# meilisearch/arroy

Measured on AMD Instinct MI355X. Metric: distances/sec, Q=1 batched 768-dim cosine scan (GB/s vs HBM roofline in `roofline`); tree-build seconds at 10M vectors in `build_10m`, higher is better.
Workload: dtype f32; 1 GPU; 1M x 768 cosine Q=1 scan (configs[1])

## Files before the change

### arroy_amd/csrc/api.hip

```cpp
#include <algorithm>
#include <atomic>
#include <chrono>
#include <cmath>
#include <condition_variable>
#include <functional>
#include <immintrin.h>
#include <new>
#include <thread>
#include <cctype>
#include <cstdio>
#include <mutex>
#include <vector>
#include <sched.h>
#include <sys/syscall.h>
#include <unistd.h>

#include "common.h"

namespace ah {

static thread_local std::string g_error;
static thread_local ah_error_detail g_detail = {AH_OK, 0, 0, 0};

static thread_local int g_guard_depth = 0;
// ... 1998 lines not shown
        std::lock_guard<std::mutex> lk(ds->mu);
        ah_rerank_stats &r = ds->rr_stats;
        r.calls += 1;
        r.queries += nq;
        r.candidates += total;
        r.seconds_wall += wall;
        r.seconds_prep += prep;
        r.seconds_ids += ids;
        r.seconds_enqueue += enqueue;
        r.seconds_sync_wait += wait;
        r.seconds_device_span += ms * 1e-3;
    }
};
#define AH_RR_SYNC(stream_)                       \
    do {                                          \
        probe.lap(&RerankProbe::enqueue);         \
        AH_HIP(hipStreamSynchronize(stream_));    \
        probe.lap(&RerankProbe::wait);            \
    } while (0)

static int rerank_batch_chunk(ah_dataset *ds, Context *ctx, const float *queries, size_t nq, const uint32_t *ids,
                              const uint64_t *offsets, size_t k, uint32_t *out_ids, float *out_distances,
                              uint32_t *out_counts) {
    const uint64_t base = offsets[0];
    const uint64_t total = offsets[nq] - base;
    RerankProbe probe(ds, ctx, nq, total);
    uint32_t max_n = 0, max_rounds = 0;
    std::vector<HostSeg> segs(nq);
    std::vector<HostTile> tiles;
    const uint32_t tc = batch_tile_candidates();
    for (size_t q = 0; q < nq; q++) {
        const uint64_t nq_items = offsets[q + 1] - offsets[q];
        AH_REQUIRE(nq_items < 0xFFFFFFFFull, AH_ERR_INVALID_ARGUMENT, "candidate list too long");
        segs[q] = HostSeg{offsets[q] - base, (uint32_t)nq_items, (uint32_t)std::min<uint64_t>(k, nq_items)};
        out_counts[q] = segs[q].k;
        max_n = std::max(max_n, segs[q].n);
        max_rounds = std::max(max_rounds, batch_rounds(segs[q].n, segs[q].k));
        for (uint32_t f = 0; f < segs[q].n; f += tc) tiles.push_back(HostTile{(uint32_t)q, f});
    }
    const size_t qstride = pad256(ds->row_bytes());
    const size_t kstride = batch_key_stride(std::max<uint32_t>(max_n, 1));
    const size_t inv_bytes = batch_invert_wanted(ds->view(), total) ? batch_invert_counter_bytes(ds->n, total) : 0;
    bool screened = tun(TUN_RERANK_SCREEN) != 0 && (ds->metric == AH_COSINE || ds->metric == AH_DOT_PRODUCT) && ds->dims >= 32 &&
                    inv_bytes == 0 && k <= 256 && total >= 8 * k * nq && !tiles.empty();
    if (screened) screened = ensure_screen(ds, ctx->stream, false);
    const bool screened8 = screened && tun(TUN_RERANK_SCREEN8) != 0 && !ds->rerank8_off.load(std::memory_order_relaxed) &&
                           ensure_screen8_search(ds, ctx->stream);
    const size_t screen_bytes = (screened ? pad256(nq * (size_t)ds->hpitch * 2) + pad256(nq * 16) + pad256(total * 4) : 0) +
                                (screened8 ? pad256(nq * (size_t)ds->pitch8 * 2) + pad256(nq * 16) + pad256(total * 4) : 0);
    const size_t dev_bytes = pad256(nq * (size_t)ds->dims * 4) + nq * qstride + pad256(nq * 8) + pad256(nq * sizeof(HostSeg)) +
                             pad256(tiles.size() * sizeof(HostTile)) + pad256(total * 4) * 2 + 2 * pad256(nq * kstride * 8) +
                             pad256(nq * k * 4) * 2 + pad256(inv_bytes) + screen_bytes + 4096;
    const size_t pin_bytes = pad256(nq * (size_t)ds->dims * 4) + pad256(nq * sizeof(HostSeg)) +
                             pad256(tiles.size() * sizeof(HostTile)) + pad256(total * 4) + pad256(nq * k * 4) * 2 + 4096;
    AH_TRY(ctx->ensure_device(dev_bytes));
    AH_TRY(ctx->ensure_pinned(pin_bytes));
    Carver dev(ctx->d_scratch), pin(ctx->h_pinned);
    float *d_qf32 = dev.take<float>(nq * (size_t)ds->dims);
    uint8_t *d_qvecs = dev.take<uint8_t>(nq * qstride);
    float *d_qhdrs = dev.take<float>(nq * 2);
    HostSeg *d_segs = dev.take<HostSeg>(nq);
    HostTile *d_tiles = dev.take<HostTile>(tiles.size());
    uint32_t *d_ids = dev.take<uint32_t>(total);
    float *d_dist = dev.take<float>(total);
    uint64_t *d_ka = dev.take<uint64_t>(nq * kstride);
    uint64_t *d_kb = dev.take<uint64_t>(nq * kstride);
    uint32_t *d_oi = dev.take<uint32_t>(nq * k);
    float *d_od = dev.take<float>(nq * k);
    uint32_t *d_err = dev.take<uint32_t>(16);
    uint32_t *d_inv = inv_bytes ? dev.take<uint32_t>(inv_bytes / 4) : nullptr;
    uint16_t *d_q16 = screened ? dev.take<uint16_t>(nq * (size_t)ds->hpitch) : nullptr;
    float4 *d_qstats = screened ? dev.take<float4>(nq) : nullptr;
    float *d_aux = screened ? dev.take<float>(total) : nullptr;
    int8_t *d_q8 = screened8 ? dev.take<int8_t>(nq * (size_t)ds->pitch8 * 2) : nullptr;
    float4 *d_q8stats = screened8 ? dev.take<float4>(nq) : nullptr;
    float *d_aux8 = screened8 ? dev.take<float>(total) : nullptr;
    float *h_q = pin.take<float>(nq * (size_t)ds->dims);
    HostSeg *h_segs = pin.take<HostSeg>(nq);
    HostTile *h_tiles = pin.take<HostTile>(tiles.size());
    uint32_t *h_ids = pin.take<uint32_t>(total);
    uint32_t *h_oi = pin.take<uint32_t>(nq * k);
    float *h_od = pin.take<float>(nq * k);
    uint32_t *h_err = pin.take<uint32_t>(16);
    bool retried8 = false;
    auto note_screened = [&](const uint32_t *words) {
        std::lock_guard<std::mutex> lk(ds->mu);
        ds->rr_stats.queries_screened += words[9];
        ds->rr_stats.survivors += words[10];
        ds->rr_stats.chunks_int8 += screened8 && !retried8 ? 1 : 0;
    };
    auto retry_on_binary16 = [&](uint32_t err_bits) -> int {
        if (!screened8) return AH_OK;
        const bool overflow = (err_bits & ~1u) == 8u;
        if (screen8_window_note(ds->rerank8_seen, ds->rerank8_fails, overflow)) ds->rerank8_off.store(true, std::memory_order_relaxed);
        if (!overflow) return AH_OK;
        retried8 = true;
        {
            std::lock_guard<std::mutex> lk(ds->mu);
            ds->rr_stats.chunks_int8_retried += 1;
        }
        AH_HIP(hipMemsetAsync(d_err, 0, 64, ctx->stream));
        AH_TRY(launch_rerank_screened(ds, (uint32_t)nq, d_qvecs, qstride, d_qhdrs, d_segs, d_tiles, 0u, (uint32_t)tiles.size(), tc, d_ids,
                                      d_dist, d_aux, d_q16, d_qstats, (uint32_t)k, d_oi, d_od, d_err, ctx->stream, true, true));
        AH_HIP(hipMemcpyAsync(h_oi, d_oi, nq * k * 4, hipMemcpyDeviceToHost, ctx->stream));
        AH_HIP(hipMemcpyAsync(h_od, d_od, nq * k * 4, hipMemcpyDeviceToHost, ctx->stream));
        AH_HIP(hipMemcpyAsync(h_err, d_err, 64, hipMemcpyDeviceToHost, ctx->stream));
        AH_HIP(hipStreamSynchronize(ctx->stream));
        return AH_OK;
    };
    memcpy(h_q, queries, nq * (size_t)ds->dims * 4);
    memcpy(h_segs, segs.data(), nq * sizeof(HostSeg));
    if (!tiles.empty()) memcpy(h_tiles, tiles.data(), tiles.size() * sizeof(HostTile));
    hipStream_t s = ctx->stream;
    probe.lap(&RerankProbe::prep);
    probe.first_enqueue(s);
    AH_HIP(hipMemcpyAsync(d_qf32, h_q, nq * (size_t)ds->dims * 4, hipMemcpyHostToDevice, s));
    AH_HIP(hipMemcpyAsync(d_segs, h_segs, nq * sizeof(HostSeg), hipMemcpyHostToDevice, s));
    if (!tiles.empty()) AH_HIP(hipMemcpyAsync(d_tiles, h_tiles, tiles.size() * sizeof(HostTile), hipMemcpyHostToDevice, s));
    AH_HIP(hipMemsetAsync(d_err, 0, 64, s));
    const uint64_t n_groups = (uint64_t)std::max<long long>(1, tun(TUN_RERANK_GROUPS));
    const bool pipelined = screened && n_groups > 1 && total >= (512u << 10);
    if (pipelined && !ctx->copy_stream && create_copy_stream(&ctx->copy_stream) != hipSuccess) {
        (void)hipGetLastError();
        ctx->copy_stream = nullptr;
    }
    if (pipelined && ctx->copy_stream) {
        AH_TRY(launch_prepare_queries_only(ds->view(), d_qf32, (uint32_t)nq, d_qvecs, qstride, d_qhdrs, s));
        const uint64_t group_ids = (total + n_groups - 1) / n_groups;
        size_t qa = 0;
        uint32_t ta = 0;
        bool first = true;
        while (qa < nq) {
            size_t qb = qa + 1;
            while (qb < nq && segs[qb].off + segs[qb].n - segs[qa].off <= group_ids) qb++;
            const uint64_t lo = segs[qa].off, len = segs[qb - 1].off + segs[qb - 1].n - lo;
            uint32_t tb = ta;
            while (tb < tiles.size() && tiles[tb].query < qb) tb++;
            if (len) {
                probe.lap(&RerankProbe::enqueue);
                parallel_rows(len, 4, [&](size_t a, size_t b) { memcpy(h_ids + lo + a, ids + base + lo + a, (b - a) * 4); });
                probe.lap(&RerankProbe::ids);
                AH_HIP(hipMemcpyAsync(d_ids + lo, h_ids + lo, len * 4, hipMemcpyHostToDevice, ctx->copy_stream));
                AH_HIP(hipEventRecord(ctx->ev0, ctx->copy_stream));
                AH_HIP(hipStreamWaitEvent(s, ctx->ev0, 0));
            }
            AH_TRY(launch_rerank_screened(ds, (uint32_t)nq, d_qvecs, qstride, d_qhdrs, d_segs, d_tiles, ta, tb - ta, tc, d_ids, d_dist,
                                          d_aux, d_q16, d_qstats, (uint32_t)k, d_oi, d_od, d_err, s, first, qb == nq, d_q8, d_q8stats,
                                          d_aux8));
            first = false;
            qa = qb;
            ta = tb;
        }
        AH_HIP(hipMemcpyAsync(h_oi, d_oi, nq * k * 4, hipMemcpyDeviceToHost, s));
        AH_HIP(hipMemcpyAsync(h_od, d_od, nq * k * 4, hipMemcpyDeviceToHost, s));
        AH_HIP(hipMemcpyAsync(h_err, d_err, 64, hipMemcpyDeviceToHost, s));
        AH_RR_SYNC(s);
        AH_TRY(check_err_flags(*h_err, true));
        AH_TRY(retry_on_binary16(*h_err));
        if ((*h_err & ~1u) == 0) {
            note_screened(h_err);
            AH_TRY(check_err_flags(*h_err, true));
            memcpy(out_ids, h_oi, nq * k * 4);
            memcpy(out_distances, h_od, nq * k * 4);
            return AH_OK;
        }
        AH_HIP(hipMemsetAsync(d_err, 0, 64, s));
        AH_TRY(launch_rerank_batch_prepared(ds->view(), (uint32_t)nq, d_qvecs, qstride, d_qhdrs, d_segs, d_tiles, (uint32_t)tiles.size(),
                                            d_ids, d_dist, d_ka, d_kb, kstride, max_n, (uint32_t)k, max_rounds, d_oi, d_od, d_err, s,
                                            total, d_inv));
        AH_HIP(hipMemcpyAsync(h_oi, d_oi, nq * k * 4, hipMemcpyDeviceToHost, s));
        AH_HIP(hipMemcpyAsync(h_od, d_od, nq * k * 4, hipMemcpyDeviceToHost, s));
        AH_HIP(hipMemcpyAsync(h_err, d_err, 64, hipMemcpyDeviceToHost, s));
        AH_RR_SYNC(s);
        AH_TRY(check_err_flags(*h_err, true));
        memcpy(out_ids, h_oi, nq * k * 4);
        memcpy(out_distances, h_od, nq * k * 4);
        return AH_OK;
    }
    for (uint64_t lo = 0; lo < total; lo += (2u << 20)) {
        const uint64_t len = std::min<uint64_t>(2u << 20, total - lo);
        probe.lap(&RerankProbe::enqueue);
        parallel_rows(len, 4, [&](size_t a, size_t b) { memcpy(h_ids + lo + a, ids + base + lo + a, (b - a) * 4); });
        probe.lap(&RerankProbe::ids);
        AH_HIP(hipMemcpyAsync(d_ids + lo, h_ids + lo, len * 4, hipMemcpyHostToDevice, s));
    }
    if (screened) {
        AH_TRY(launch_prepare_queries_only(ds->view(), d_qf32, (uint32_t)nq, d_qvecs, qstride, d_qhdrs, s));
        AH_TRY(launch_rerank_screened(ds, (uint32_t)nq, d_qvecs, qstride, d_qhdrs, d_segs, d_tiles, 0u, (uint32_t)tiles.size(), tc, d_ids,
                                      d_dist, d_aux, d_q16, d_qstats, (uint32_t)k, d_oi, d_od, d_err, s, true, true, d_q8, d_q8stats, d_aux8));
        AH_HIP(hipMemcpyAsync(h_oi, d_oi, nq * k * 4, hipMemcpyDeviceToHost, s));
        AH_HIP(hipMemcpyAsync(h_od, d_od, nq * k * 4, hipMemcpyDeviceToHost, s));
        AH_HIP(hipMemcpyAsync(h_err, d_err, 64, hipMemcpyDeviceToHost, s));
        AH_RR_SYNC(s);
        AH_TRY(check_err_flags(*h_err, true));
        AH_TRY(retry_on_binary16(*h_err));
        if ((*h_err & ~1u) == 0) {
            note_screened(h_err);
            AH_TRY(check_err_flags(*h_err, true));
            memcpy(out_ids, h_oi, nq * k * 4);
            memcpy(out_distances, h_od, nq * k * 4);
            return AH_OK;
        }
        AH_HIP(hipMemsetAsync(d_err, 0, 64, s));
        AH_TRY(launch_rerank_batch_prepared(ds->view(), (uint32_t)nq, d_qvecs, qstride, d_qhdrs, d_segs, d_tiles, (uint32_t)tiles.size(),
                                            d_ids, d_dist, d_ka, d_kb, kstride, max_n, (uint32_t)k, max_rounds, d_oi, d_od, d_err, s,
                                            total, d_inv));
    } else {
        AH_TRY(launch_rerank_batch(ds->view(), d_qf32, (uint32_t)nq, d_qvecs, qstride, d_qhdrs, d_segs, d_tiles,
                                   (uint32_t)tiles.size(), d_ids, d_dist, d_ka, d_kb, kstride, max_n, (uint32_t)k, max_rounds,
                                   d_oi, d_od, d_err, s, total, d_inv));
    }
    AH_HIP(hipMemcpyAsync(h_oi, d_oi, nq * k * 4, hipMemcpyDeviceToHost, s));
    AH_HIP(hipMemcpyAsync(h_od, d_od, nq * k * 4, hipMemcpyDeviceToHost, s));
    AH_HIP(hipMemcpyAsync(h_err, d_err, 64, hipMemcpyDeviceToHost, s));
    AH_RR_SYNC(s);
    AH_TRY(check_err_flags(*h_err, true));
    memcpy(out_ids, h_oi, nq * k * 4);
    memcpy(out_distances, h_od, nq * k * 4);
    return AH_OK;
}

int ah_rerank_batch(ah_dataset *ds, const float *queries, size_t n_queries, const uint32_t *ids,
                    const uint64_t *offsets, size_t k, uint32_t *out_ids, float *out_distances, uint32_t *out_counts) {
    AH_GUARDED("ah_rerank_batch")
    AH_NEED_FINALIZED(ds);
    AH_REQUIRE(queries && ids && offsets && out_ids && out_distances && out_counts, AH_ERR_INVALID_ARGUMENT,
               "NULL argument");
    if (n_queries == 0) return AH_OK;
    AH_REQUIRE(k > 0, AH_ERR_INVALID_ARGUMENT, "k must be > 0");
    for (size_t q = 0; q < n_queries; q++)
        AH_REQUIRE(offsets[q + 1] >= offsets[q], AH_ERR_INVALID_ARGUMENT, "offsets must be non-decreasing");
    if (!batch_supported((uint32_t)std::min<size_t>(k, 0xFFFFFFFFu))) {
        for (size_t q = 0; q < n_queries; q++) {
            for (size_t t = 0; t < k; t++) {
                out_ids[q * k + t] = 0xFFFFFFFFu;
                uint32_t nan_bits = 0xFFFFFFFFu;
                memcpy(&out_distances[q * k + t], &nan_bits, 4);
            }
            size_t got = 0;
            const size_t nq_items = offsets[q + 1] - offsets[q];
            out_counts[q] = 0;
            if (nq_items == 0) continue;
            AH_TRY(ah_rerank_by_vector(ds, queries + q * (size_t)ds->dims, ids + offsets[q], nq_items, k, out_ids + q * k,
                                       out_distances + q * k, &got));
            out_counts[q] = (uint32_t)got;
        }
        return AH_OK;
    }
    AH_LEASE(ds, ctx);
    size_t q0 = 0;
    while (q0 < n_queries) {
        size_t q1 = q0 + 1;
        while (q1 < n_queries && q1 - q0 < 1024 && offsets[q1 + 1] - offsets[q0] <= (64ull << 20)) q1++;
        AH_TRY(rerank_batch_chunk(ds, ctx, queries + q0 * (size_t)ds->dims, q1 - q0, ids, offsets + q0, k, out_ids + q0 * k,
                                  out_distances + q0 * k, out_counts + q0));
        q0 = q1;
    }
    return AH_OK;
    AH_GUARDED_END
}

int ah_dataset_rerank_stats(ah_dataset *ds, ah_rerank_stats *out, int reset) {
    AH_GUARDED("ah_dataset_rerank_stats")
    AH_REQUIRE(ds, AH_ERR_INVALID_ARGUMENT, "dataset is NULL");
    std::lock_guard<std::mutex> lk(ds->mu);
    if (out) *out = ds->rr_stats;
    if (reset) ds->rr_stats = ah_rerank_stats{};
// ... 281 lines not shown
```

### arroy_amd/csrc/common.h

```cpp
#pragma once

#include <hip/hip_runtime.h>

#include <cstdarg>
#include <cstdint>
#include <cstdio>
#include <atomic>
#include <cstring>
#include <mutex>
#include <new>
#include <string>
#include <thread>
#include <vector>

#include "../../include/arroy_hip.h"
#include "../../include/arroy_hip_policy.h"

namespace ah {

void set_error(const char *fmt, ...);
const char *last_error();
void set_error_status(int status);
void set_error_detail(uint32_t item, uint64_t expected, uint64_t received);

// ... 73 lines not shown
    X(SCREEN, "AH_SCREEN", 1)                             \
    X(SCREEN_VERIFY, "AH_SCREEN_VERIFY", 0)       \
    X(NODE_PREFETCH, "AH_NODE_PREFETCH", 1)         \
    X(SCREEN8_LO, "AH_SCREEN8_LO", 1)                 \
    X(SCREEN8, "AH_SCREEN8", -1)                 \
    X(MASK_BITS, "AH_MASK_BITS", -1)             \
    X(DENSE, "AH_DENSE", -1)                        \
    X(DENSE_MAX_COLS, "AH_DENSE_MAX_COLS", 16384)                                                                        \
    X(DENSE_NARROW, "AH_DENSE_NARROW", -1)               \
    X(DENSE_NARROW_MAX_COLS, "AH_DENSE_NARROW_MAX_COLS", 64)    \
    X(DENSE_NARROW_STREAM, "AH_DENSE_NARROW_STREAM", 0)  \
    X(DENSE_GMACS, "AH_DENSE_GMACS", 495000)           \
    X(MARGIN_MODE, "AH_MARGIN_MODE", 0)                          \
    X(READBACK_DIRECT, "AH_READBACK_DIRECT", 0)              \
    X(READBACK_PRIORITY, "AH_READBACK_PRIORITY", 1)  \
    X(READBACK_MB, "AH_READBACK_MB", 256)        \
    X(NUMA, "AH_NUMA", 1)                        \
    X(RETRY_GATE, "AH_RETRY_GATE", 1)            \
    X(TAIL_GROUPS, "AH_BUILD_TAIL_GROUPS", 5)    \
    X(TAIL_MIN_MB, "AH_BUILD_TAIL_MIN_MB", 64)   \
    X(TAIL_NODE_ITEMS, "AH_BUILD_TAIL_NODE_ITEMS", 2)  \
    X(TAIL_RATIO, "AH_BUILD_TAIL_RATIO", 76)     \
    X(SCAN_BLOCKS, "AH_SCAN_BLOCKS", 0)                                 \
    X(SCAN_PACKED, "AH_SCAN_PACKED", -1)         \
    X(SCAN_GRID, "AH_SCAN_GRID", 1)              \
    X(MANHATTAN_ROWS, "AH_MANHATTAN_ROWS", 1)                                                                            \
    X(RERANK_INVERT, "AH_RERANK_INVERT", -1)          \
    X(RERANK_SMALL, "AH_RERANK_SMALL", 1)        \
    X(PAIR_GROUP, "AH_PAIR_GROUP", 0)                                                                                    \
    X(PAIR_RUNS, "AH_PAIR_RUNS", 1)                                                                                      \
    X(SEARCH_BITMAP, "AH_SEARCH_BITMAP", 1)          \
    X(SEARCH_TILES, "AH_SEARCH_TILES", 1)                          \
    X(SEARCH_WAVE, "AH_SEARCH_WAVE", 1)                        \
    X(SEARCH_BLOCK_MAX_QUERIES, "AH_SEARCH_BLOCK_MAX_QUERIES", 64)  \
    X(SEARCH_SMALL_GATE, "AH_SEARCH_SMALL_GATE", 1)  \
    X(SEARCH_SMALL_UNITS_MAX_QUERIES, "AH_SEARCH_SMALL_UNITS_MAX_QUERIES", 64)  \
    X(SEARCH_FUSED_FLAG, "AH_SEARCH_FUSED_FLAG", 1)  \
    X(SEARCH_FUSED_PREPARE, "AH_SEARCH_FUSED_PREPARE", 1)  \
    X(SEARCH_SINGLE_FUSED, "AH_SEARCH_SINGLE_FUSED", 1)  \
    X(SEARCH_SMALL_TILES_MAX_QUERIES, "AH_SEARCH_SMALL_TILES_MAX_QUERIES", 8)  \
    X(SEARCH_MULTI, "AH_SEARCH_MULTI", 1)        \
    X(SEARCH_MULTI_TREES_PER_BLOCK, "AH_SEARCH_MULTI_TREES_PER_BLOCK", 8)  \
    X(SEARCH_MULTI_IDS_BY_TILES, "AH_SEARCH_MULTI_IDS_BY_TILES", 1)  \
    X(SEARCH_SPIN_WAIT, "AH_SEARCH_SPIN_WAIT", 1)  \
    X(SEARCH_FLAT_TILES, "AH_SEARCH_FLAT_TILES", 1)  \
    X(SEARCH_STATUS_WIPE, "AH_SEARCH_STATUS_WIPE", 1)  \
    X(SEARCH_ITEM_LIST, "AH_SEARCH_ITEM_LIST", 1)  \
    X(SEARCH_MULTI_OWN_UNITS, "AH_SEARCH_MULTI_OWN_UNITS", 1)  \
    X(SEARCH_MULTI_TRACE, "AH_SEARCH_MULTI_TRACE", 0)  \
    X(SEARCH_MULTI_MAX_QUERIES, "AH_SEARCH_MULTI_MAX_QUERIES", 32)  \
    X(EXACT_WIDE, "AH_EXACT_WIDE", 1)            \
    X(RERANK_GROUPS, "AH_RERANK_GROUPS", 2)      \
    X(RERANK_SCREEN8, "AH_RERANK_SCREEN8", 1)    \
    X(SEARCH_SCREEN8_MAX_VISITS, "AH_SEARCH_SCREEN8_MAX_VISITS", 4)  \
    X(SEARCH_SCREEN8_MIN_QUERIES, "AH_SEARCH_SCREEN8_MIN_QUERIES", 65)  \
    X(SEARCH_SCREEN8, "AH_SEARCH_SCREEN8", 1)    \
    X(RERANK_SCREEN, "AH_RERANK_SCREEN", 1)      \
    X(REPLICATE_HOST_BOUNCE, "AH_REPLICATE_HOST_BOUNCE", 0)  \
    X(RERANK_TIMING, "AH_RERANK_TIMING", 0)      \
    X(SEARCH_SCREEN, "AH_SEARCH_SCREEN", 1)      \
    X(SEARCH_FILTER_GROUP_MIN, "AH_SEARCH_FILTER_GROUP_MIN", 16)  \
    X(HOST_THREADS, "AH_HOST_THREADS", 8)               \
    X(DEVICE_CACHE_MB, "AH_DEVICE_CACHE_MB", 98304)  \
    X(HOST_CACHE_MB, "AH_HOST_CACHE_MB", 16384)    \
    X(CACHE_KEEP_IDLE, "AH_CACHE_KEEP_IDLE", 0)  \
    X(FAIL_ALLOC_AFTER, "AH_FAIL_ALLOC_AFTER", 0)  \
    X(STAGE_THREADS, "AH_STAGE_THREADS", 0)                                                                              \
    X(STAGE_MEMCPY, "AH_STAGE_MEMCPY", 0)                                                                                \
    X(STAGE_REGISTER, "AH_STAGE_REGISTER", 0)
enum Tunable {
#define AH_X(id, name, def) TUN_##id,
    AH_TUNABLES(AH_X)
#undef AH_X
        TUN_COUNT
};
long long tun(int id);

template <class F>
inline void parallel_run(unsigned n, F fn) {
    std::vector<std::thread> pool;
    unsigned started = 1;
    try {
        pool.reserve(n);
        for (; started < n; started++) pool.emplace_back(fn, started);
    } catch (...) {
    }
    if (n) fn(0u);
    for (unsigned t = started; t < n; t++) fn(t);
    for (auto &th : pool) th.join();
}

hipError_t dev_malloc(void **p, size_t bytes, bool optional = false);
template <typename T>
inline hipError_t dev_malloc(T **p, size_t bytes, bool optional = false) {
    return dev_malloc(reinterpret_cast<void **>(p), bytes, optional);
}
void dataset_born(int device);
void dataset_gone(int device);
size_t host_cache_trim();
hipError_t create_copy_stream(hipStream_t *out);
int numa_node_of_device(int device);
bool numa_bind_thread_to_node(int node);
void numa_prefer_node(void *p, size_t bytes, int node);
void pinned_spare_fill(int device, size_t bytes);
size_t pinned_spare_trim();
size_t dev_cache_live_bytes(int device);
// ... 291 lines not shown
```

### arroy_amd/csrc/search.hip

```cpp
#include <algorithm>
#include <chrono>
#include <memory>
#include <new>

#include "common.h"
#include "index_device.h"
#include "split_device.h"
#include "screen_device.h"

namespace ah {

static constexpr uint32_t kHeapLds = 1024;
static constexpr uint32_t kSortLds = 16384;

struct Visit {
    uint32_t node;
    uint32_t q;
    uint32_t pos;
    uint32_t n;
};
struct VisitSink {
    Visit *visits;
    uint32_t *total;
    uint32_t cap;
// ... 2039 lines not shown
                                                    const TileUnit *__restrict__ units, const uint32_t *__restrict__ n_units_p,
                                                    const uint8_t *__restrict__ qvecs, uint64_t qstride,
                                                    const float *__restrict__ qhdrs, float *__restrict__ dist, uint32_t stride,
                                                    uint32_t *err) {
    extern __shared__ uint4 s_ring4[];
    uint8_t *ring = reinterpret_cast<uint8_t *>(s_ring4);
    const uint32_t n_units = *n_units_p;
    for (uint32_t u = blockIdx.x; u < n_units; u += gridDim.x) {
        const TileUnit unit = units[u];
        const Visit *vis = sorted + unit.first;
        const uint32_t n_leaf = vis[0].n;
        const uint32_t n_vis = unit.n_vis, slab = n_vis > 8 ? kTileSlab : 2 * kTileSlab;
        const uint32_t row_begin = blockIdx.y * slab;
        if (row_begin >= n_leaf) continue;
        const uint32_t row_end = min(n_leaf, row_begin + slab);
        const uint32_t *leaf_ids = nns + (uint64_t)vis[0].q * stride + vis[0].pos;
#define AH_TILE(R, Q, QO) \
    leaf_tile<METRIC, R, Q, QO>(dv, leaf_ids, row_begin, row_end, vis, n_vis, qvecs, qstride, qhdrs, dist, stride, err)
#define AH_RING(QO, DEPTH) \
    leaf_tile_ring<METRIC, QO, DEPTH>(dv, leaf_ids, row_begin, row_end, vis, n_vis, qvecs, qstride, qhdrs, dist, stride, err, ring)
        if (n_vis > 8) AH_RING(4, 6);
        else if (n_vis > 4) AH_RING(2, 6);
        else if (n_vis > 2) AH_TILE(4, 4, 1);
        else if (n_vis == 2) AH_TILE(4, 2, 1);
        else AH_TILE(8, 1, 1);
#undef AH_TILE
#undef AH_RING
    }
}

struct PairSeg {
    uint64_t off;
    uint32_t n, k;
};
struct PairTile {
    uint32_t query, first;
};
struct ScreenSearch {
    const uint16_t *rows16;
    float4 max_stats;
    float *aux;
    uint32_t hpitch;
    float gamma_s, gamma_r;
    const uint16_t *q16;
    const float4 *qstats;
    const int8_t *rows8;
    const float *row_scale8;
    const float *dim_scale;
    uint32_t pitch8;
    float4 max8;
    const int8_t *q8;
    const float4 *q8stats;
    float *aux8;
};

__device__ __forceinline__ void query_i8(uint32_t q, uint32_t lane, const uint8_t *__restrict__ qvecs, uint64_t qstride, uint32_t dims,
                                         const ScreenSearch &ss, float gamma_r) {
    const float *v = reinterpret_cast<const float *>(qvecs + (uint64_t)q * qstride);
    int8_t *out_hi = const_cast<int8_t *>(ss.q8) + (uint64_t)q * 2 * ss.pitch8, *out_lo = out_hi + ss.pitch8;
    uint32_t mbits = 0;
    for (uint32_t i = lane; i < dims; i += 64) mbits = max(mbits, __float_as_uint(v[i] * ss.dim_scale[i]) & 0x7FFFFFFFu);
    for (int off = 32; off > 0; off >>= 1) mbits = max(mbits, (uint32_t)__shfl_xor((int)mbits, off));
    const float m = __uint_as_float(mbits);
    const bool ok = mbits >= kTinyBits && mbits < 0x7F800000u;
    const float scale = ok ? m / 127.0f : 0.0f, inv_scale = ok ? 127.0f / m : 0.0f;
    float sa = 0.f, sb = 0.f, sc = 0.f, s0 = 0.f;
    for (uint32_t i = lane; i < ss.pitch8; i += 64) {
        const float x0 = i < dims ? v[i] : 0.0f;
        const float x = i < dims ? x0 * ss.dim_scale[i] : 0.0f;
        const float t = x * inv_scale;
        const int qh = ok ? quantize8(x, inv_scale) : 0;
        const int ql = ok ? (int)fminf(fmaxf(rintf((t - (float)qh) * 256.0f), -127.0f), 127.0f) : 0;
        const float y = ((float)qh + (float)ql * 0.00390625f) * scale, d = x - y;
        sa += y * y;
        sb += d * d;
        sc += x * x;
        s0 += x0 * x0;
        out_hi[i] = (int8_t)qh;
        out_lo[i] = (int8_t)ql;
    }
    for (int off = 32; off > 0; off >>= 1) {
        sa += __shfl_xor(sa, off);
        sb += __shfl_xor(sb, off);
        sc += __shfl_xor(sc, off);
        s0 += __shfl_xor(s0, off);
    }
    if (lane == 0) {
        const float up = 1.0f + (float)(ss.pitch8 + 64u) * 1.2e-7f;
        const float inf = __uint_as_float(0x7F800000u);
        const float an = sqrtf(sa) * up, cn = sqrtf(sc) * up, cn0 = sqrtf(s0) * up;
        const float bn = ok ? sqrtf(sb) * up + 128.0f * scale * 6.0e-8f * sqrtf((float)ss.pitch8) : (mbits == 0u ? 0.0f : inf);
        const float a = (bn * ss.max8.x + cn * ss.max8.y + 2.0e-6f * (an * ss.max8.x) + gamma_r * (cn0 * ss.max8.z)) * 1.000001f * 1.002f;
        const_cast<float4 *>(ss.q8stats)[q] = make_float4(scale, a, 0.0f, 0.0f);
    }
}
__global__ __launch_bounds__(64) void k_queries_i8(const uint8_t *__restrict__ qvecs, uint64_t qstride, uint32_t dims, ScreenSearch ss) {
    query_i8(blockIdx.x, threadIdx.x, qvecs, qstride, dims, ss, ss.gamma_r);
}

template <int R, int Q, int QO, int KF = 1>
__device__ __forceinline__ void leaf_tile16(const ScreenSearch &ss, const DataView &dv, const uint32_t *__restrict__ leaf_ids,
                                            uint32_t row_begin, uint32_t n_rows, const Visit *__restrict__ vis, uint32_t n_vis,
                                            float *__restrict__ dist, uint32_t stride, uint32_t *err, uint32_t *__restrict__ copy_ids_to = nullptr,
                                            const Visit *only_visit = nullptr) {
    constexpr uint32_t RO = 8 / QO;
    const uint32_t j = threadIdx.x & 7u, ow = (threadIdx.x >> 3) & 7u, wave = threadIdx.x >> 6;
// ... 551 lines not shown
#pragma unroll
    for (uint32_t r = 0; r < kOwn; r++)
        if (own_ok >> r & 1u) atomicAdd(&s_hist[bin_of(own_u[r])], 1u);
    AH_SELECT_REST(g, id, uk, lk, atomicAdd(&s_hist[bin_of(uk)], 1u))
    __syncthreads();
    {
        constexpr uint32_t kPer = kBins / kThreads;
        uint32_t c[kPer], mine = 0;
#pragma unroll
        for (uint32_t u = 0; u < kPer; u++) {
            c[u] = s_hist[tid * kPer + u];
            mine += c[u];
        }
        uint32_t incl = mine;
        for (int off = 1; off < 64; off <<= 1) {
            const uint32_t up = __shfl_up(incl, off);
            if ((int)(tid & 63u) >= off) incl += up;
        }
        if ((tid & 63u) == 63u) s_wave[tid >> 6] = incl;
        __syncthreads();
        uint32_t before = incl - mine;
        for (uint32_t w = 0; w < (tid >> 6); w++) before += s_wave[w];
#pragma unroll
        for (uint32_t u = 0; u < kPer; u++) {
            if (before < kk && before + c[u] >= kk) s_bin = tid * kPer + u;
            before += c[u];
        }
    }
    __syncthreads();
    stamp(4);
    const uint32_t bin_k = s_bin;
    uint32_t t_key;
    if (direct) {
        t_key = w_min + bin_k;
    } else {
        const uint64_t lim = ((uint64_t)bin_k + 1ull) << 32;
        const uint64_t d = (lim + scale - 1ull) / scale;
        t_key = (uint32_t)min((uint64_t)w_min + d - 1ull, (uint64_t)s_max);
    }
#pragma unroll
    for (uint32_t r = 0; r < kOwn; r++)
        if ((own_ok >> r & 1u) && own_l[r] <= t_key) {
            const uint32_t at = atomicAdd(&s_n, 1u);
            if (at < kCap) s_pos[at] = own_id[r];
        }
    AH_SELECT_REST(g, id, uk, lk, if (lk <= t_key) {
        const uint32_t at = atomicAdd(&s_n, 1u);
        if (at < kCap) s_pos[at] = id;
    })
#undef AH_SELECT_REST
    __syncthreads();
    stamp(5);
    const uint32_t n_sel = s_n;
    if (n_sel > kCap) {
        if (tid == 0) atomicOr(err, 8u);
        return;
    }
    if (tid == 0) {
        atomicAdd(&err[SS_SCREENED], 1u);
        atomicAdd(&err[SS_SURVIVORS], n_sel);
    }
    const uint32_t j = tid & 7u;
    bool bad = false;
    for (uint32_t e = tid >> 3; e < n_sel; e += kThreads >> 3) {
        const uint32_t id = s_pos[e];
        const uint64_t row = row_of_id(dv, id);
        const float xh = METRIC == AH_COSINE ? dv.headers[row] : 0.0f;
        const float r = octet_reduce_stream<OP_DOT, 16, true>(s_qf4, dv.rows_f32 + row * dv.pitch, dv.dims, j);
        const float d = METRIC == AH_COSINE ? cosine_from_dot(r, qn, xh) : -r;
        if (j == 0) {
            const uint32_t w = orderable_key(d);
            if (w > 0xFF7FFFFFu) bad = true;
            s_key[e] = ((uint64_t)w << 32) | id;
            s_val[e] = d;
        }
    }
    if (bad) atomicOr(err, 4u);
    __syncthreads();
    stamp(6);
    for (uint32_t e = tid; e < n_sel; e += kThreads) {
        const uint64_t mine = s_key[e];
        uint32_t rank = 0;
        uint32_t i = 0;
        for (; i + 8 <= n_sel; i += 8) {
            uint64_t other[8];
#pragma unroll
            for (uint32_t u = 0; u < 8; u++) other[u] = s_key[i + u];
#pragma unroll
            for (uint32_t u = 0; u < 8; u++) rank += (other[u] < mine || (other[u] == mine && i + u < e)) ? 1u : 0u;
        }
        for (; i < n_sel; i++) {
            const uint64_t other = s_key[i];
            rank += (other < mine || (other == mine && i < e)) ? 1u : 0u;
        }
        if (rank < kk) {
            out_ids[(uint64_t)q * k_out + rank] = (uint32_t)mine;
            out_dist[(uint64_t)q * k_out + rank] = normalized_distance(dv.metric, s_val[e], dv.dims);
        }
    }
    stamp(7);
    if (trace && threadIdx.x == 0 && blockIdx.x == 0) trace[9] = n_sel;
}

template <int METRIC, bool FLAG = false>
__global__ __launch_bounds__(1024) void k_search_select_screened(DataView dv, ScreenSearch ss, const uint32_t *__restrict__ nns,
                                                                 const float *__restrict__ dist_all, uint32_t stride,
                                                                 const uint32_t *__restrict__ counts,
// ... 325 lines not shown
    }
    uint32_t node = live ? roots[t] : 0u;
    while (__any(active)) {
        if (!active) continue;
        const DNode nd = nodes[node];
        if ((nd.kind & 0xFFu) == AH_NODE_DESCENDANTS) {
            if (j == 0) out_leaf[pair] = node;
            active = false;
            continue;
        }
        uint32_t right;
        if (nd.kind & 0x100u) right = side_of_margin(descent_margin(nv, nd.c, leaf_vec, lh, j));
        else right = ah_route_side_is_left(seeds[t], rank ? rank[node] : node, id) ^ 1u;
        node = right ? nd.b : nd.a;
    }
}

__global__ __launch_bounds__(256) void k_filter_stored(DataView dv, const uint32_t *__restrict__ ids, uint64_t n,
                                                       unsigned long long *__restrict__ out) {
    const uint64_t stride = (uint64_t)gridDim.x * blockDim.x;
    uint32_t c = 0;
    for (uint64_t g = (uint64_t)blockIdx.x * blockDim.x + threadIdx.x; g < n; g += stride) c += row_of_id(dv, ids[g]) != ~0ull ? 1u : 0u;
    for (uint32_t d = 32; d > 0; d >>= 1) c += __shfl_xor(c, d, 64);
    if ((threadIdx.x & 63u) == 0 && c) atomicAdd(out, (unsigned long long)c);
}

__global__ void k_unpack_normals(const uint8_t *__restrict__ recs, const uint64_t *__restrict__ offsets, uint32_t n,
                                 uint64_t vec_off, uint64_t hdr_off, uint32_t valid_words32, uint32_t row_words32,
                                 uint32_t hf, uint32_t *__restrict__ rows, float *__restrict__ headers) {
    const uint32_t r = blockIdx.x;
    if (r >= n) return;
    const uint32_t *src = reinterpret_cast<const uint32_t *>(recs + offsets[r] + vec_off);
    for (uint32_t i = threadIdx.x; i < row_words32; i += blockDim.x)
        rows[(uint64_t)r * row_words32 + i] = i < valid_words32 ? src[i] : 0u;
    if (threadIdx.x < hf)
        headers[(uint64_t)r * hf + threadIdx.x] = reinterpret_cast<const float *>(recs + offsets[r] + hdr_off)[threadIdx.x];
}

int launch_rerank_screened(ah_dataset *ds, uint32_t nq, const uint8_t *d_qvecs, uint64_t qstride, const float *d_qhdrs,
                           const void *d_segs, const void *d_tiles, uint32_t tile_first, uint32_t n_tiles, uint32_t tile_candidates,
                           const uint32_t *d_ids, float *d_dist, float *d_aux, uint16_t *d_q16, float4 *d_qstats, uint32_t k_out,
                           uint32_t *d_out_ids, float *d_out_dist, uint32_t *d_err, hipStream_t s, bool first, bool select,
                           int8_t *d_q8, float4 *d_q8stats, float *d_aux8) {
    const DataView dv = ds->view();
    ScreenSearch ss{};
    ss.rows16 = ds->d_rows_h16;
    ss.max_stats = make_float4(ds->screen_max[0], ds->screen_max[1], ds->screen_max[2], 0.0f);
    ss.aux = ds->metric == AH_COSINE ? d_aux : nullptr;
    ss.hpitch = ds->hpitch;
    ss.gamma_s = (float)(4.0 * (2.0 * (ds->hpitch / 16) + 8.0) * 5.9604645e-8);
    ss.gamma_r = (float)(4.0 * ((double)(ds->dims / 32) + 6.0 + 62.0) * 5.9604645e-8);
    ss.q16 = d_q16;
    ss.qstats = d_qstats;
    if (d_q8) {
        ss.rows8 = ds->d_rows_i8;
        ss.row_scale8 = ds->d_scale8_rows;
        ss.dim_scale = ds->d_dim_scale;
        ss.pitch8 = ds->pitch8;
        ss.max8 = make_float4(ds->screen8_max[0], ds->screen8_max[1], ds->screen8_max[2], 0.0f);
        ss.q8 = d_q8;
        ss.q8stats = d_q8stats;
        ss.aux8 = d_aux8;
        ss.qstats = nullptr;
        if (first) hipLaunchKernelGGL(k_queries_i8, dim3(nq), dim3(64), 0, s, d_qvecs, qstride, ds->dims, ss);
        const size_t sh8 = (size_t)ds->pitch8 * 2;
        if (sh8 > 48 * 1024)
            AH_HIP(hipFuncSetAttribute(reinterpret_cast<const void *>(k_pairs_screen8), hipFuncAttributeMaxDynamicSharedMemorySize, (int)sh8));
        if (n_tiles)
            hipLaunchKernelGGL(k_pairs_screen8, dim3(n_tiles), dim3(256), sh8, s, dv, ss, reinterpret_cast<const PairSeg *>(d_segs),
                               reinterpret_cast<const PairTile *>(d_tiles) + tile_first, tile_candidates, d_ids, d_dist, d_err);
    } else {
        if (first) hipLaunchKernelGGL(k_queries_h16, dim3(nq), dim3(64), 0, s, d_qvecs, qstride, ds->dims, ds->hpitch, d_q16, d_qstats);
        const size_t sh = (size_t)ds->hpitch * 2;
        if (sh > 48 * 1024)
            AH_HIP(hipFuncSetAttribute(reinterpret_cast<const void *>(k_pairs_screen16), hipFuncAttributeMaxDynamicSharedMemorySize, (int)sh));
        if (n_tiles)
            hipLaunchKernelGGL(k_pairs_screen16, dim3(n_tiles), dim3(256), sh, s, dv, ss, reinterpret_cast<const PairSeg *>(d_segs),
                               reinterpret_cast<const PairTile *>(d_tiles) + tile_first, tile_candidates, d_ids, d_dist, d_err);
    }
    if (!select) {
        AH_HIP(hipGetLastError());
        return AH_OK;
    }
    AH_TRY(launch_screen_verify(ds, ss, d_ids, d_dist, 0u, nullptr, reinterpret_cast<const PairSeg *>(d_segs), nq, d_qvecs, qstride,
                                d_qhdrs, s));
    const size_t sel_lds = (size_t)ds->pitch * 4;
    if (sel_lds > 32 * 1024) {
        AH_HIP(hipFuncSetAttribute(reinterpret_cast<const void *>(k_search_select_screened<AH_COSINE>),
                                   hipFuncAttributeMaxDynamicSharedMemorySize, (int)sel_lds));
        AH_HIP(hipFuncSetAttribute(reinterpret_cast<const void *>(k_search_select_screened<AH_DOT_PRODUCT>),
                                   hipFuncAttributeMaxDynamicSharedMemorySize, (int)sel_lds));
    }
    if (ds->metric == AH_COSINE)
        hipLaunchKernelGGL((k_search_select_screened<AH_COSINE>), dim3(nq), dim3(1024), sel_lds, s, dv, ss, d_ids, d_dist, 0u,
                           (const uint32_t *)nullptr, (const uint32_t *)nullptr, k_out, d_qvecs, qstride, d_qhdrs, d_out_ids,
                           d_out_dist, d_err, reinterpret_cast<const PairSeg *>(d_segs));
    else
        hipLaunchKernelGGL((k_search_select_screened<AH_DOT_PRODUCT>), dim3(nq), dim3(1024), sel_lds, s, dv, ss, d_ids, d_dist, 0u,
                           (const uint32_t *)nullptr, (const uint32_t *)nullptr, k_out, d_qvecs, qstride, d_qhdrs, d_out_ids,
                           d_out_dist, d_err, reinterpret_cast<const PairSeg *>(d_segs));
    AH_HIP(hipGetLastError());
    return AH_OK;
}

void index_prepare_screens(ah_dataset *ds) {
    if (tun(TUN_SEARCH_SCREEN) != 0 && (ds->metric == AH_COSINE || ds->metric == AH_DOT_PRODUCT) && ds->dims >= 32 && ds->n) {
// ... 1305 lines not shown
```

Before: 3.063 billion distances/s.

## Coalesce rerank uploads/downloads into single contiguous copies and prefetch next id group

Reorders device scratch carving so the output ids, distances and error words sit contiguously, letting one device-to-host copy replace three. Likewise the error-zeroing, query, segment and tile uploads become one host-to-device copy from a matching pinned block, replacing separate memcpys and a memset. The pipelined path precomputes balanced id groups, launches the query prep step before any wait on ids, and enqueues the next group's id copy after the current kernel so host staging overlaps device work. It also adds a tunable selection cap, which at its default leaves behaviour unchanged. The main risk is the contiguous-layout assumption if the carver pads between allocations (it copies the padding too) and reuse of a single event across groups.

```diff
diff --git a/arroy_amd/csrc/api.hip b/arroy_amd/csrc/api.hip
--- a/arroy_amd/csrc/api.hip
+++ b/arroy_amd/csrc/api.hip
@@ -2074,22 +2074,24 @@
                              pad256(tiles.size() * sizeof(HostTile)) + pad256(total * 4) * 2 + 2 * pad256(nq * kstride * 8) +
                              pad256(nq * k * 4) * 2 + pad256(inv_bytes) + screen_bytes + 4096;
     const size_t pin_bytes = pad256(nq * (size_t)ds->dims * 4) + pad256(nq * sizeof(HostSeg)) +
-                             pad256(tiles.size() * sizeof(HostTile)) + pad256(total * 4) + pad256(nq * k * 4) * 2 + 4096;
+                             pad256(tiles.size() * sizeof(HostTile)) + pad256(total * 4) + pad256(nq * k * 4) * 2 + 256 + 4096;
     AH_TRY(ctx->ensure_device(dev_bytes));
     AH_TRY(ctx->ensure_pinned(pin_bytes));
     Carver dev(ctx->d_scratch), pin(ctx->h_pinned);
+    uint32_t *d_oi = dev.take<uint32_t>(nq * k);
+    float *d_od = dev.take<float>(nq * k);
+    uint32_t *d_err = dev.take<uint32_t>(16);
     float *d_qf32 = dev.take<float>(nq * (size_t)ds->dims);
+    HostSeg *d_segs = dev.take<HostSeg>(nq);
+    HostTile *d_tiles = dev.take<HostTile>(tiles.size());
+    const size_t out_block = (size_t)((uint8_t *)(d_err + 16) - (uint8_t *)d_oi);
+    const size_t in_block = (size_t)((dev.base + dev.off) - (uint8_t *)d_err);
     uint8_t *d_qvecs = dev.take<uint8_t>(nq * qstride);
     float *d_qhdrs = dev.take<float>(nq * 2);
-    HostSeg *d_segs = dev.take<HostSeg>(nq);
-    HostTile *d_tiles = dev.take<HostTile>(tiles.size());
     uint32_t *d_ids = dev.take<uint32_t>(total);
     float *d_dist = dev.take<float>(total);
     uint64_t *d_ka = dev.take<uint64_t>(nq * kstride);
     uint64_t *d_kb = dev.take<uint64_t>(nq * kstride);
-    uint32_t *d_oi = dev.take<uint32_t>(nq * k);
-    float *d_od = dev.take<float>(nq * k);
-    uint32_t *d_err = dev.take<uint32_t>(16);
     uint32_t *d_inv = inv_bytes ? dev.take<uint32_t>(inv_bytes / 4) : nullptr;
     uint16_t *d_q16 = screened ? dev.take<uint16_t>(nq * (size_t)ds->hpitch) : nullptr;
     float4 *d_qstats = screened ? dev.take<float4>(nq) : nullptr;
@@ -2097,13 +2099,18 @@
     int8_t *d_q8 = screened8 ? dev.take<int8_t>(nq * (size_t)ds->pitch8 * 2) : nullptr;
     float4 *d_q8stats = screened8 ? dev.take<float4>(nq) : nullptr;
     float *d_aux8 = screened8 ? dev.take<float>(total) : nullptr;
+    uint32_t *h_oi = pin.take<uint32_t>(nq * k);
+    float *h_od = pin.take<float>(nq * k);
+    uint32_t *h_err = pin.take<uint32_t>(16);
+    uint32_t *h_zero = pin.take<uint32_t>(16);
     float *h_q = pin.take<float>(nq * (size_t)ds->dims);
     HostSeg *h_segs = pin.take<HostSeg>(nq);
     HostTile *h_tiles = pin.take<HostTile>(tiles.size());
     uint32_t *h_ids = pin.take<uint32_t>(total);
-    uint32_t *h_oi = pin.take<uint32_t>(nq * k);
-    float *h_od = pin.take<float>(nq * k);
-    uint32_t *h_err = pin.take<uint32_t>(16);
+    auto fetch_results = [&]() -> int {
+        AH_HIP(hipMemcpyAsync(h_oi, d_oi, out_block, hipMemcpyDeviceToHost, ctx->stream));
+        return AH_OK;
+    };
     bool retried8 = false;
     auto note_screened = [&](const uint32_t *words) {
         std::lock_guard<std::mutex> lk(ds->mu);
@@ -2124,22 +2131,21 @@
         AH_HIP(hipMemsetAsync(d_err, 0, 64, ctx->stream));
         AH_TRY(launch_rerank_screened(ds, (uint32_t)nq, d_qvecs, qstride, d_qhdrs, d_segs, d_tiles, 0u, (uint32_t)tiles.size(), tc, d_ids,
                                       d_dist, d_aux, d_q16, d_qstats, (uint32_t)k, d_oi, d_od, d_err, ctx->stream, true, true));
-        AH_HIP(hipMemcpyAsync(h_oi, d_oi, nq * k * 4, hipMemcpyDeviceToHost, ctx->stream));
-        AH_HIP(hipMemcpyAsync(h_od, d_od, nq * k * 4, hipMemcpyDeviceToHost, ctx->stream));
-        AH_HIP(hipMemcpyAsync(h_err, d_err, 64, hipMemcpyDeviceToHost, ctx->stream));
+        AH_TRY(fetch_results());
         AH_HIP(hipStreamSynchronize(ctx->stream));
         return AH_OK;
     };
-    memcpy(h_q, queries, nq * (size_t)ds->dims * 4);
-    memcpy(h_segs, segs.data(), nq * sizeof(HostSeg));
-    if (!tiles.empty()) memcpy(h_tiles, tiles.data(), tiles.size() * sizeof(HostTile));
     hipStream_t s = ctx->stream;
-    probe.lap(&RerankProbe::prep);
-    probe.first_enqueue(s);
-    AH_HIP(hipMemcpyAsync(d_qf32, h_q, nq * (size_t)ds->dims * 4, hipMemcpyHostToDevice, s));
-    AH_HIP(hipMemcpyAsync(d_segs, h_segs, nq * sizeof(HostSeg), hipMemcpyHostToDevice, s));
-    if (!tiles.empty()) AH_HIP(hipMemcpyAsync(d_tiles, h_tiles, tiles.size() * sizeof(HostTile), hipMemcpyHostToDevice, s));
-    AH_HIP(hipMemsetAsync(d_err, 0, 64, s));
+    auto upload_inputs = [&](bool span_starts_here) -> int {
+        memset(h_zero, 0, 64);
+        memcpy(h_q, queries, nq * (size_t)ds->dims * 4);
+        memcpy(h_segs, segs.data(), nq * sizeof(HostSeg));
+        if (!tiles.empty()) memcpy(h_tiles, tiles.data(), tiles.size() * sizeof(HostTile));
+        probe.lap(&RerankProbe::prep);
+        if (span_starts_here) probe.first_enqueue(s);
+        AH_HIP(hipMemcpyAsync(d_err, h_zero, in_block, hipMemcpyHostToDevice, s));
+        return AH_OK;
+    };
     const uint64_t n_groups = (uint64_t)std::max<long long>(1, tun(TUN_RERANK_GROUPS));
     const bool pipelined = screened && n_groups > 1 && total >= (512u << 10);
     if (pipelined && !ctx->copy_stream && create_copy_stream(&ctx->copy_stream) != hipSuccess) {
@@ -2147,35 +2153,56 @@
         ctx->copy_stream = nullptr;
     }
     if (pipelined && ctx->copy_stream) {
+        struct Group {
+            size_t qb;
+            uint32_t tb;
+            uint64_t lo, len;
+        };
+        std::vector<Group> groups;
+        {
+            size_t qa = 0;
+            uint32_t ta = 0;
+            while (qa < nq) {
+                size_t qb = nq;
+                if (groups.size() + 1 < n_groups) {
+                    const uint64_t bound = total / n_groups * (groups.size() + 1);
+                    qb = qa + 1;
+                    while (qb < nq && segs[qb].off + segs[qb].n <= bound) qb++;
+                }
+                const uint64_t lo = segs[qa].off;
+                uint32_t tb = ta;
+                while (tb < tiles.size() && tiles[tb].query < qb) tb++;
+                groups.push_back(Group{qb, tb, lo, segs[qb - 1].off + segs[qb - 1].n - lo});
+                qa = qb;
+                ta = tb;
+            }
+        }
+        auto send_ids = [&](const Group &g) -> int {
+            if (g.len == 0) return AH_OK;
+            probe.lap(&RerankProbe::enqueue);
+            parallel_rows(g.len, 4, [&](size_t a, size_t b) { memcpy(h_ids + g.lo + a, ids + base + g.lo + a, (b - a) * 4); });
+            probe.lap(&RerankProbe::ids);
+            AH_HIP(hipMemcpyAsync(d_ids + g.lo, h_ids + g.lo, g.len * 4, hipMemcpyHostToDevice, ctx->copy_stream));
+            AH_HIP(hipEventRecord(ctx->ev0, ctx->copy_stream));
+            return AH_OK;
+        };
+        probe.lap(&RerankProbe::prep);
+        probe.first_enqueue(s);
+        AH_TRY(send_ids(groups[0]));
+        AH_TRY(upload_inputs(false));
         AH_TRY(launch_prepare_queries_only(ds->view(), d_qf32, (uint32_t)nq, d_qvecs, qstride, d_qhdrs, s));
-        const uint64_t group_ids = (total + n_groups - 1) / n_groups;
-        size_t qa = 0;
+        AH_TRY(launch_rerank_screened(ds, (uint32_t)nq, d_qvecs, qstride, d_qhdrs, d_segs, d_tiles, 0u, 0u, tc, d_ids, d_dist, d_aux, d_q16,
+                                      d_qstats, (uint32_t)k, d_oi, d_od, d_err, s, true, false, d_q8, d_q8stats, d_aux8));
         uint32_t ta = 0;
-        bool first = true;
-        while (qa < nq) {
-            size_t qb = qa + 1;
-            while (qb < nq && segs[qb].off + segs[qb].n - segs[qa].off <= group_ids) qb++;
-            const uint64_t lo = segs[qa].off, len = segs[qb - 1].off + segs[qb - 1].n - lo;
-            uint32_t tb = ta;
-            while (tb < tiles.size() && tiles[tb].query < qb) tb++;
-            if (len) {
-                probe.lap(&RerankProbe::enqueue);
-                parallel_rows(len, 4, [&](size_t a, size_t b) { memcpy(h_ids + lo + a, ids + base + lo + a, (b - a) * 4); });
-                probe.lap(&RerankProbe::ids);
-                AH_HIP(hipMemcpyAsync(d_ids + lo, h_ids + lo, len * 4, hipMemcpyHostToDevice, ctx->copy_stream));
-                AH_HIP(hipEventRecord(ctx->ev0, ctx->copy_stream));
-                AH_HIP(hipStreamWaitEvent(s, ctx->ev0, 0));
-            }
-            AH_TRY(launch_rerank_screened(ds, (uint32_t)nq, d_qvecs, qstride, d_qhdrs, d_segs, d_tiles, ta, tb - ta, tc, d_ids, d_dist,
-                                          d_aux, d_q16, d_qstats, (uint32_t)k, d_oi, d_od, d_err, s, first, qb == nq, d_q8, d_q8stats,
-                                          d_aux8));
-            first = false;
-            qa = qb;
-            ta = tb;
-        }
-        AH_HIP(hipMemcpyAsync(h_oi, d_oi, nq * k * 4, hipMemcpyDeviceToHost, s));
-        AH_HIP(hipMemcpyAsync(h_od, d_od, nq * k * 4, hipMemcpyDeviceToHost, s));
-        AH_HIP(hipMemcpyAsync(h_err, d_err, 64, hipMemcpyDeviceToHost, s));
+        for (size_t g = 0; g < groups.size(); g++) {
+            if (groups[g].len) AH_HIP(hipStreamWaitEvent(s, ctx->ev0, 0));
+            AH_TRY(launch_rerank_screened(ds, (uint32_t)nq, d_qvecs, qstride, d_qhdrs, d_segs, d_tiles, ta, groups[g].tb - ta, tc, d_ids,
+                                          d_dist, d_aux, d_q16, d_qstats, (uint32_t)k, d_oi, d_od, d_err, s, false, g + 1 == groups.size(),
+                                          d_q8, d_q8stats, d_aux8));
+            ta = groups[g].tb;
+            if (g + 1 < groups.size()) AH_TRY(send_ids(groups[g + 1]));
+        }
+        AH_TRY(fetch_results());
         AH_RR_SYNC(s);
         AH_TRY(check_err_flags(*h_err, true));
         AH_TRY(retry_on_binary16(*h_err));
@@ -2190,15 +2217,14 @@
         AH_TRY(launch_rerank_batch_prepared(ds->view(), (uint32_t)nq, d_qvecs, qstride, d_qhdrs, d_segs, d_tiles, (uint32_t)tiles.size(),
                                             d_ids, d_dist, d_ka, d_kb, kstride, max_n, (uint32_t)k, max_rounds, d_oi, d_od, d_err, s,
                                             total, d_inv));
-        AH_HIP(hipMemcpyAsync(h_oi, d_oi, nq * k * 4, hipMemcpyDeviceToHost, s));
-        AH_HIP(hipMemcpyAsync(h_od, d_od, nq * k * 4, hipMemcpyDeviceToHost, s));
-        AH_HIP(hipMemcpyAsync(h_err, d_err, 64, hipMemcpyDeviceToHost, s));
+        AH_TRY(fetch_results());
         AH_RR_SYNC(s);
         AH_TRY(check_err_flags(*h_err, true));
         memcpy(out_ids, h_oi, nq * k * 4);
         memcpy(out_distances, h_od, nq * k * 4);
         return AH_OK;
     }
+    AH_TRY(upload_inputs(true));
     for (uint64_t lo = 0; lo < total; lo += (2u << 20)) {
         const uint64_t len = std::min<uint64_t>(2u << 20, total - lo);
         probe.lap(&RerankProbe::enqueue);
@@ -2210,9 +2236,7 @@
         AH_TRY(launch_prepare_queries_only(ds->view(), d_qf32, (uint32_t)nq, d_qvecs, qstride, d_qhdrs, s));
         AH_TRY(launch_rerank_screened(ds, (uint32_t)nq, d_qvecs, qstride, d_qhdrs, d_segs, d_tiles, 0u, (uint32_t)tiles.size(), tc, d_ids,
                                       d_dist, d_aux, d_q16, d_qstats, (uint32_t)k, d_oi, d_od, d_err, s, true, true, d_q8, d_q8stats, d_aux8));
-        AH_HIP(hipMemcpyAsync(h_oi, d_oi, nq * k * 4, hipMemcpyDeviceToHost, s));
-        AH_HIP(hipMemcpyAsync(h_od, d_od, nq * k * 4, hipMemcpyDeviceToHost, s));
-        AH_HIP(hipMemcpyAsync(h_err, d_err, 64, hipMemcpyDeviceToHost, s));
+        AH_TRY(fetch_results());
         AH_RR_SYNC(s);
         AH_TRY(check_err_flags(*h_err, true));
         AH_TRY(retry_on_binary16(*h_err));
@@ -2232,9 +2256,7 @@
                                    (uint32_t)tiles.size(), d_ids, d_dist, d_ka, d_kb, kstride, max_n, (uint32_t)k, max_rounds,
                                    d_oi, d_od, d_err, s, total, d_inv));
     }
-    AH_HIP(hipMemcpyAsync(h_oi, d_oi, nq * k * 4, hipMemcpyDeviceToHost, s));
-    AH_HIP(hipMemcpyAsync(h_od, d_od, nq * k * 4, hipMemcpyDeviceToHost, s));
-    AH_HIP(hipMemcpyAsync(h_err, d_err, 64, hipMemcpyDeviceToHost, s));
+    AH_TRY(fetch_results());
     AH_RR_SYNC(s);
     AH_TRY(check_err_flags(*h_err, true));
     memcpy(out_ids, h_oi, nq * k * 4);
diff --git a/arroy_amd/csrc/common.h b/arroy_amd/csrc/common.h
--- a/arroy_amd/csrc/common.h
+++ b/arroy_amd/csrc/common.h
@@ -149,6 +149,7 @@
     X(EXACT_WIDE, "AH_EXACT_WIDE", 1)            \
     X(RERANK_GROUPS, "AH_RERANK_GROUPS", 2)      \
     X(RERANK_SCREEN8, "AH_RERANK_SCREEN8", 1)    \
+    X(RERANK_SELECT_CAP, "AH_RERANK_SELECT_CAP", 1024)  \
     X(SEARCH_SCREEN8_MAX_VISITS, "AH_SEARCH_SCREEN8_MAX_VISITS", 4)  \
     X(SEARCH_SCREEN8_MIN_QUERIES, "AH_SEARCH_SCREEN8_MIN_QUERIES", 65)  \
     X(SEARCH_SCREEN8, "AH_SEARCH_SCREEN8", 1)    \
diff --git a/arroy_amd/csrc/search.hip b/arroy_amd/csrc/search.hip
--- a/arroy_amd/csrc/search.hip
+++ b/arroy_amd/csrc/search.hip
@@ -2115,6 +2115,7 @@
     const int8_t *q8;
     const float4 *q8stats;
     float *aux8;
+    uint32_t sel_cap;
 };
 
 __device__ __forceinline__ void query_i8(uint32_t q, uint32_t lane, const uint8_t *__restrict__ qvecs, uint64_t qstride, uint32_t dims,
@@ -2772,7 +2773,7 @@
     __syncthreads();
     stamp(5);
     const uint32_t n_sel = s_n;
-    if (n_sel > kCap) {
+    if (n_sel > (ss.sel_cap ? ss.sel_cap : kCap)) {
         if (tid == 0) atomicOr(err, 8u);
         return;
     }
@@ -3204,6 +3205,8 @@
     ss.gamma_r = (float)(4.0 * ((double)(ds->dims / 32) + 6.0 + 62.0) * 5.9604645e-8);
     ss.q16 = d_q16;
     ss.qstats = d_qstats;
+    const long long cap = tun(TUN_RERANK_SELECT_CAP);
+    ss.sel_cap = cap >= 1 && cap < 1024 ? (uint32_t)cap : 0u;
     if (d_q8) {
         ss.rows8 = ds->d_rows_i8;
         ss.row_scale8 = ds->d_scale8_rows;
```

New measurement: 3.056 billion distances/s. Within noise of the previous version (-0.2%).
